# NethermindEth/zinc

Hardware: AMD Instinct MI355X
Metric: Zip commit+open MCoeffs/s at 2^24 witness (higher is better)
Workload: dtype i64

## Files before the change

zinc_amd/csrc/kernels_commit.cuh:

```cuda
#pragma once
#include <hip/hip_runtime.h>
#include <stdint.h>

#include "blake3.cuh"

namespace zipk {

typedef __int128 i128;
typedef unsigned __int128 u128;

#ifdef ZIPK_DEBUG_STAMPS
constexpr uint32_t kStampRec = 64;
__device__ __forceinline__ unsigned long long stamp_hw_id() {
    const uint32_t xcc = __builtin_amdgcn_s_getreg((3 << 11) | 20), hw = __builtin_amdgcn_s_getreg((31 << 11) | 4);
    return (unsigned long long)xcc | ((unsigned long long)hw << 8);
}
#endif

struct CommitArgs {
    const int64_t *evals;
    const uint32_t *perm1;
    const uint32_t *perm2;
    uint64_t *rows;
    uint32_t compact_rows;
    uint32_t *layers;
    uint32_t *roots;
    uint32_t row_len;
    uint32_t cw;
    uint32_t nact;
    uint32_t num_rows;
    uint32_t rounds_per_chunk;
    uint64_t chunk_ends;
    uint8_t *pk;
    uint32_t pk_stride, pk_off0, pk_off1, pk_off2;
    const uint32_t *pk_tab;
    uint32_t *chunk_done;
    uint32_t classes;
    const uint32_t *need;
    unsigned long long *clock;
    uint4 *slab;
#ifdef ZIPK_DEBUG_STAMPS
    unsigned long long *stamps;
#endif
};

__device__ __forceinline__ i128 shfl_up_i96(i128 x, int off) {
    uint32_t d0 = (uint32_t)x, d1 = (uint32_t)((u128)x >> 32), d2 = (uint32_t)((u128)x >> 64);
    d0 = __shfl_up(d0, off, 64);
    d1 = __shfl_up(d1, off, 64);
    d2 = __shfl_up(d2, off, 64);
    const int64_t hi = (int64_t)(int32_t)d2;
    return (i128)(((u128)(uint64_t)hi << 64) | ((u128)d1 << 32) | d0);
}

__device__ __forceinline__ void lds_barrier() {
    asm volatile("s_waitcnt lgkmcnt(0)\n\ts_barrier" ::: "memory");
}

template <int CTRL, int ROW_MASK>
__device__ __forceinline__ i128 dpp_i96(i128 x) {
    const int d0 = (int)(uint32_t)x, d1 = (int)(uint32_t)((u128)x >> 32), d2 = (int)(uint32_t)((u128)x >> 64);
    const uint32_t y0 = (uint32_t)__builtin_amdgcn_update_dpp(0, d0, CTRL, ROW_MASK, 0xF, false);
    const uint32_t y1 = (uint32_t)__builtin_amdgcn_update_dpp(0, d1, CTRL, ROW_MASK, 0xF, false);
    const uint32_t y2 = (uint32_t)__builtin_amdgcn_update_dpp(0, d2, CTRL, ROW_MASK, 0xF, false);
    const int64_t hi = (int64_t)(int32_t)y2;
    return (i128)(((u128)(uint64_t)hi << 64) | ((u128)y1 << 32) | y0);
}

__device__ __forceinline__ i128 block_exclusive_scan_i96(i128 total, i128 *wave_tot, int which) {
    const int lane = threadIdx.x & 63;
    const int wid = __builtin_amdgcn_readfirstlane((int)(threadIdx.x >> 6));
    i128 x = total;
    x += dpp_i96<0x111, 0xF>(x);
    x += dpp_i96<0x112, 0xF>(x);
    x += dpp_i96<0x114, 0xF>(x);
    x += dpp_i96<0x118, 0xF>(x);
    x += dpp_i96<0x142, 0xA>(x);
    x += dpp_i96<0x143, 0xC>(x);
    i128 *tot = wave_tot + 16 * which;
    if (lane == 63) tot[wid] = x;
    lds_barrier();
    i128 t = lane < 16 ? tot[lane] : (i128)0;
    t += dpp_i96<0x111, 0xF>(t);
    t += dpp_i96<0x112, 0xF>(t);
    t += dpp_i96<0x114, 0xF>(t);
    t += dpp_i96<0x118, 0xF>(t);
    i128 base = 0;
    if (wid > 0) {
        const uint32_t b0 = (uint32_t)__builtin_amdgcn_readlane((int)(uint32_t)t, wid - 1);
        const uint32_t b1 = (uint32_t)__builtin_amdgcn_readlane((int)(uint32_t)((u128)t >> 32), wid - 1);
        const uint32_t b2 = (uint32_t)__builtin_amdgcn_readlane((int)(uint32_t)((u128)t >> 64), wid - 1);
        base = (i128)(((u128)(uint64_t)(int64_t)(int32_t)b2 << 64) | ((u128)b1 << 32) | b0);
    }
    return base + (x - total);
}

__device__ __forceinline__ void store_hash(uint32_t *dst, const uint32_t (&h)[8]) {
    uint4 *d = reinterpret_cast<uint4 *>(dst);
    d[0] = make_uint4(h[0], h[1], h[2], h[3]);
    d[1] = make_uint4(h[4], h[5], h[6], h[7]);
}
__device__ __forceinline__ void load_hash(const uint32_t *src, uint32_t (&h)[8]) {
    const uint4 *s = reinterpret_cast<const uint4 *>(src);
    uint4 a = s[0], b = s[1];
    h[0] = a.x; h[1] = a.y; h[2] = a.z; h[3] = a.w;
    h[4] = b.x; h[5] = b.y; h[6] = b.z; h[7] = b.w;
}

__device__ __forceinline__ uint32_t level_off(uint32_t cw, uint32_t k) { return 2u * cw - ((2u * cw) >> k); }

template <bool ILV>
__device__ __forceinline__ uint32_t *tree_of(uint32_t *layers, uint32_t cw, uint32_t row) {
    return ILV ? layers + ((size_t)(row >> 2) * (2u * cw) * 4 + (row & 3u)) * 8 : layers + (size_t)row * (2u * cw) * 8;
}
template <bool ILV>
constexpr uint32_t kNodeWords = ILV ? 32u : 8u;

__device__ __forceinline__ uint32_t round_slot(uint32_t b, uint32_t G, uint32_t classes = 1) {
    if (G & 7u) return b;
    const uint32_t x = b & 7u, l = b >> 3;
    if (classes <= 1u) return x * (G >> 3) + l;
    const uint32_t per = (G >> 3) / classes, k = l / per;
    return k * (G / classes) + x * per + (l - k * per);
}
__device__ __forceinline__ uint32_t commit_class(uint32_t b, uint32_t G, uint32_t classes) {
    return classes <= 1u ? 0u : (b >> 3) / ((G >> 3) / classes);
}

template <int LVL, int E0, class Src>
__device__ __forceinline__ void subtree_hash(Src &src, uint32_t (&h)[8]) {
    if constexpr (LVL == 0) {
        src.template leaf<E0>(h);
    } else {
        uint32_t l[8], r[8];
        subtree_hash<LVL - 1, E0>(src, l);
        subtree_hash<LVL - 1, E0 + (1 << (LVL - 1))>(src, r);
        blake3_node(l, r, h);
        src.store(LVL, E0 >> LVL, h);
    }
}

constexpr int kStoreAll = 0, kStoreHinted = 1, kStorePacked = 3;

template <int E, int MODE = kStoreAll, bool LAZY = false>
struct StridedLeaves {
    static constexpr bool MASKED = MODE != kStoreAll;
    uint32_t w0[E], w1[E], w2[E];
    const uint64_t *lz_lo = nullptr;
    const uint32_t *lz_hi = nullptr;
    uint32_t lz_stride = 0;
    template <int E0>
    __device__ __forceinline__ void entry(uint32_t &a, uint32_t &b, uint32_t &c) const {
        if (LAZY) {
            const uint64_t lo = lz_lo[E0 * lz_stride];
            a = (uint32_t)lo;
            b = (uint32_t)(lo >> 32);
            c = lz_hi[E0 * lz_stride];
        } else {
            a = w0[E0];
            b = w1[E0];
            c = w2[E0];
        }
    }
    uint64_t *out_row;
    uint32_t *tree;
    uint32_t cw, T, tid;
    uint32_t base = 0;
    uint32_t compact = 0;
    uint32_t smask = 0xFFFFFFFFu;
    static constexpr uint32_t NW = MODE == kStorePacked ? 32u : 8u;
    uint8_t *pk_v = nullptr, *pk_n = nullptr;
    uint32_t pk_off0 = 0, pk_off1 = 0, pk_off2 = 0;
    __device__ __forceinline__ void set_packed(const CommitArgs &a, uint32_t row) {
        uint8_t *g = a.pk + (size_t)(row >> 2) * 4 * a.pk_stride;
        pk_v = g + (row & 3u) * 16u;
        pk_n = g + (row & 3u) * 32u;
        pk_off0 = 4u * a.pk_off0;
        pk_off1 = 4u * a.pk_off1;
        pk_off2 = 4u * a.pk_off2;
    }
    uint32_t ptab[16] = {};
    template <int K>
    __device__ __forceinline__ uint32_t pbase() const { return (ptab[K >> 1] >> ((K & 1) * 16)) & 0xFFFFu; }
    static __device__ __forceinline__ uint32_t lanes_below(uint64_t m) {
        return __builtin_amdgcn_mbcnt_hi((uint32_t)(m >> 32), __builtin_amdgcn_mbcnt_lo((uint32_t)m, 0u));
    }
    template <int E0>
    __device__ __forceinline__ void store_row_of(uint32_t d0, uint32_t d1, uint32_t d2) {
        if (MASKED && !(smask & (1u << E0))) return;
        const uint32_t j = base + E0 * T + tid;
        const uint32_t s = (uint32_t)((int32_t)d2 >> 31);
        if (MODE == kStorePacked) {
            const uint32_t pos = pbase<E0>() + lanes_below(__builtin_amdgcn_ballot_w64(true));
            *reinterpret_cast<uint4 *>(pk_v + (size_t)pos * 64) = make_uint4(d0, d1, d2, s);
        } else if (compact) {
            *reinterpret_cast<uint4 *>(out_row + (size_t)j * 2) = make_uint4(d0, d1, d2, s);
        } else {
            uint4 *o = reinterpret_cast<uint4 *>(out_row + (size_t)j * 4);
            o[0] = make_uint4(d0, d1, d2, s);
            o[1] = make_uint4(s, s, s, s);
        }
    }
    template <int E0>
    __device__ __forceinline__ void store_row() {
        uint32_t d0, d1, d2;
        entry<E0>(d0, d1, d2);
        store_row_of<E0>(d0, d1, d2);
    }
    template <int E0>
    __device__ __forceinline__ void leaf(uint32_t (&h)[8]) {
        uint32_t d0, d1, d2;
        entry<E0>(d0, d1, d2);
        store_row_of<E0>(d0, d1, d2);
        blake3_leaf_sext96(d0, d1, d2, h);
        if (!MASKED || (smask & (0x100u << E0))) {
            if (MODE == kStorePacked) {
                const uint32_t pos = pbase<8 + E0>() + lanes_below(__builtin_amdgcn_ballot_w64(true));
                store_hash(reinterpret_cast<uint32_t *>(pk_n + pk_off0) + (size_t)pos * 32, h);
            } else {
                store_hash(tree + (size_t)(base + E0 * T + tid) * 8, h);
            }
        }
    }
    template <int LVL, int E0>
    __device__ __forceinline__ void store(const uint32_t (&h)[8]) {
        if (MASKED && LVL <= 2 && !(smask & ((LVL == 1 ? 0x10000u : 0x1000000u) << (E0 >> LVL)))) return;
        const uint32_t e = E0 + (tid & ((1u << LVL) - 1u));
        const uint32_t n = (base + e * T + tid) >> LVL;
        if (MODE == kStorePacked && LVL == 1) {
            const uint64_t act = __builtin_amdgcn_ballot_w64(true);
            const bool odd = tid & 1u;
            const uint32_t pos = (odd ? pbase<16 + (E0 >> 1) * 2 + 1>() : pbase<16 + (E0 >> 1) * 2>()) +
                                 lanes_below(act & (odd ? 0xAAAAAAAAAAAAAAAAull : 0x5555555555555555ull));
            store_hash(reinterpret_cast<uint32_t *>(pk_n + pk_off1) + (size_t)pos * 32, h);
        } else if (MODE == kStorePacked && LVL == 2) {
            const uint64_t act = __builtin_amdgcn_ballot_w64(true);
            const uint32_t q = tid & 3u;
            constexpr int K0 = 24 + ((E0 >> 2) & 1) * 4;
            const uint32_t b01 = (q & 1u) ? pbase<K0 + 1>() : pbase<K0>(), b23 = (q & 1u) ? pbase<K0 + 3>() : pbase<K0 + 2>();
            const uint32_t pos = ((q & 2u) ? b23 : b01) + lanes_below(act & (0x1111111111111111ull << q));
            store_hash(reinterpret_cast<uint32_t *>(pk_n + pk_off2) + (size_t)pos * 32, h);
        } else {
            store_hash(tree + ((size_t)level_off(cw, LVL) + n) * NW, h);
        }
    }
};

template <int E>
__device__ __forceinline__ uint32_t store_mask(const uint32_t *need, uint32_t cw, uint32_t base, uint32_t T, uint32_t tid) {
    if (!need) return 0xFFFFFFFFu;
    const uint32_t *nv = need, *n0 = nv + (cw + 31) / 32, *n1 = n0 + (cw + 31) / 32, *n2 = n1 + (cw / 2 + 31) / 32;
    uint32_t m = 0;
#pragma unroll
    for (int e = 0; e < E; e++) {
        const uint32_t j = base + e * T + tid;
        m |= ((nv[j >> 5] >> (j & 31)) & 1u) << e;
        m |= ((n0[j >> 5] >> (j & 31)) & 1u) << (8 + e);
    }
#pragma unroll
    for (int g = 0; g < E / 2; g++) {
        const uint32_t i = (base + (2 * g + (tid & 1u)) * T + tid) >> 1;
        m |= ((n1[i >> 5] >> (i & 31)) & 1u) << (16 + g);
    }
#pragma unroll
    for (int g = 0; g < E / 4; g++) {
        const uint32_t i = (base + (4 * g + (tid & 3u)) * T + tid) >> 2;
        m |= ((n2[i >> 5] >> (i & 31)) & 1u) << (24 + g);
    }
    return m;
}

template <int E, int E0, class Src>
__device__ __forceinline__ void store_rows_only(Src &src) {
    if constexpr (E0 < E) {
        src.template store_row<E0>();
        store_rows_only<E, E0 + 1>(src);
    }
}

template <int LVL, int E0, class Src>
__device__ __forceinline__ void bfly_hash(Src &src, uint32_t (&h)[8]) {
    if constexpr (LVL == 0) {
        src.template leaf<E0>(h);
    } else {
        uint32_t A[8], B[8], m[16];
        bfly_hash<LVL - 1, E0>(src, A);
        bfly_hash<LVL - 1, E0 + (1 << (LVL - 1))>(src, B);
        const bool up = (src.tid >> (LVL - 1)) & 1;
#pragma unroll
        for (int i = 0; i < 8; i++) {
            const uint32_t snd = up ? A[i] : B[i];
            const uint32_t rcv = __shfl_xor(snd, 1 << (LVL - 1), 64);
            m[i] = up ? rcv : A[i];
            m[8 + i] = up ? B[i] : rcv;
        }
        blake3_block64(m, h);
        src.template store<LVL, E0>(h);
    }
}

template <bool ILV>
__device__ __forceinline__ void upper_stage(const CommitArgs &a, uint32_t first, uint32_t nrows_c, uint32_t lvl, uint32_t nl,
                                            uint32_t lane, uint32_t nlanes) {
    constexpr uint32_t NW = kNodeWords<ILV>;
    const uint32_t cw = a.cw, depth = 31u - __builtin_clz(cw);
    const uint32_t u_shift = depth - (lvl - 1u) - nl;
    const uint32_t total = nrows_c << u_shift;
    const uint32_t slot0 = round_slot(blockIdx.x, gridDim.x, a.classes);
    for (uint32_t idx = lane; idx < total; idx += nlanes) {
        const uint32_t ri = idx >> u_shift, i = idx & ((1u << u_shift) - 1u);
        const uint32_t r = slot0 + (first + ri) * gridDim.x;
        uint32_t *tree = tree_of<ILV>(a.layers, cw, r);
        const uint32_t *ch = tree + ((size_t)level_off(cw, lvl - 1u) + ((size_t)i << nl)) * NW;
        uint32_t c0[8], c1[8], h0[8];
        load_hash(ch, c0);
        load_hash(ch + NW, c1);
        if (nl == 1u) {
            blake3_node(c0, c1, h0);
            store_hash(tree + ((size_t)level_off(cw, lvl) + i) * NW, h0);
            if (lvl == depth) store_hash(a.roots + (size_t)r * 8, h0);
        } else {
            uint32_t c2[8], c3[8], h1[8], h2[8];
            blake3_node(c0, c1, h0);
            uint32_t *o = tree + ((size_t)level_off(cw, lvl) + 2u * i) * NW;
            store_hash(o, h0);
            asm volatile("" ::: "memory");
            load_hash(ch + 2 * NW, c2);
            load_hash(ch + 3 * NW, c3);
            blake3_node(c2, c3, h1);
            store_hash(o + NW, h1);
            blake3_node(h0, h1, h2);
            store_hash(tree + ((size_t)level_off(cw, lvl + 1u) + i) * NW, h2);
            if (lvl + 1u == depth) store_hash(a.roots + (size_t)r * 8, h2);
        }
    }
}

struct ChunkCursor {
    uint32_t first = 0, index = 0;
    __device__ __forceinline__ bool ends_with(const CommitArgs &a, uint32_t round, bool last) const {
        if (last) return true;
        if (a.chunk_ends) return (a.chunk_ends >> round) & 1u;
        return (round + 1) % a.rounds_per_chunk == 0;
    }
    __device__ __forceinline__ void advance(uint32_t round) {
        first = round + 1;
        index++;
    }
};

constexpr uint32_t kFinisherFlagWords = 16;

template <bool HASH, bool ILV = false>
struct ChunkFinisher {
    bool pending = false;
    uint32_t p_first = 0, p_nrows = 0, p_lvl = 0, p_index = 0;
    uint32_t p_base = 0;
    uint32_t n_deferred = 0;
    uint32_t *flags = nullptr;

    __device__ __forceinline__ void init(uint32_t *lds_flags, uint32_t tid) {
        flags = lds_flags;
        if (tid < kFinisherFlagWords) lds_flags[tid] = 0;
    }

    __device__ __forceinline__ void top_of_row() const {
        if (HASH && pending) asm volatile("s_waitcnt vmcnt(0)" ::: "memory");
    }

    static __device__ __forceinline__ void publish(const CommitArgs &a, uint32_t index, uint32_t lane) {
        if (!a.chunk_done) return;
        asm volatile("s_waitcnt vmcnt(0)" ::: "memory");
        if (lane == 0) {
            __builtin_amdgcn_fence(__ATOMIC_RELEASE, "agent");
            asm volatile("s_waitcnt vmcnt(0)" ::: "memory");
            __hip_atomic_fetch_add(&a.chunk_done[index], 1u, __ATOMIC_RELAXED, __HIP_MEMORY_SCOPE_AGENT);
        }
    }

    static __device__ __forceinline__ void signal(uint32_t *flag, uint32_t lane) {
        asm volatile("s_waitcnt vmcnt(0)" ::: "memory");
        if (lane == 0) __hip_atomic_fetch_add(flag, 1u, __ATOMIC_RELEASE, __HIP_MEMORY_SCOPE_WORKGROUP);
    }
    static __device__ __forceinline__ void wait_for(uint32_t *flag, uint32_t target) {
        uint32_t spins = 0;
        while (__hip_atomic_load(flag, __ATOMIC_ACQUIRE, __HIP_MEMORY_SCOPE_WORKGROUP) < target) {
            __builtin_amdgcn_s_sleep(2);
            if (++spins > (1u << 24)) __builtin_trap();
        }
    }

    static __device__ __forceinline__ bool stage_wide(uint32_t cw, uint32_t lvl, uint32_t nl, uint32_t j) {
        return j == 0u || (cw >> (lvl - 1u + nl)) >= 64u;
    }
    static __device__ __forceinline__ uint32_t stage_waves(uint32_t cw, uint32_t depth, uint32_t lvl0, uint32_t j, uint32_t W) {
        const uint32_t lvl = lvl0 + 2u * j;
        if (lvl > depth) return 0u;
        return stage_wide(cw, lvl, depth - lvl >= 1u ? 2u : 1u, j) ? W : 1u;
    }
    __device__ __forceinline__ uint32_t target(uint32_t cw, uint32_t depth, uint32_t j, uint32_t W) const {
        return (n_deferred - 1u) * stage_waves(cw, depth, p_base, j, W) + stage_waves(cw, depth, p_lvl, j, W);
    }
    __device__ __forceinline__ void after_hash(const CommitArgs &a, uint32_t wave, uint32_t lane, uint32_t T) {
        if (!(HASH && pending)) return;
        pending = false;
        n_deferred++;
        constexpr uint32_t kFinWaves = 8u;
        const uint32_t W = T >= 64u * kFinWaves ? kFinWaves : T >= 256u ? 4u : (T + 63u) / 64u;
        if (wave >= W) return;
        const uint32_t cw = a.cw, depth = 31u - __builtin_clz(cw);
        uint32_t lvl = p_lvl, j = 0, owner = 0;
        bool wide = true;
        while (lvl <= depth) {
            const uint32_t nl = depth - lvl >= 1u ? 2u : 1u;
            wide = stage_wide(cw, lvl, nl, j);
            if (wide) {
                if (j) wait_for(flags + (j - 1u), target(cw, depth, j - 1u, W));
                upper_stage<ILV>(a, p_first, p_nrows, lvl, nl, lane + 64u * wave, 64u * W);
                signal(flags + j, lane);
            } else {
                owner = j % W;
                if (wave == owner) {
                    wait_for(flags + (j - 1u), target(cw, depth, j - 1u, W));
                    upper_stage<ILV>(a, p_first, p_nrows, lvl, nl, lane, 64u);
                    signal(flags + j, lane);
                }
            }
            lvl += nl;
            j++;
        }
        if (j == 0u || wide) owner = 0u;
        if (wave == owner) {
            if (j && wide) wait_for(flags + (j - 1u), target(cw, depth, j - 1u, W));
            publish(a, p_index, lane);
        }
    }

    __device__ __forceinline__ void after_loop(const CommitArgs &a, uint32_t wave, uint32_t lane, uint32_t T, unsigned char *lds,
                                               uint32_t lds_bytes) {
        if (!(HASH && pending)) return;
        __syncthreads();
        const uint32_t cw = a.cw, depth = 31u - __builtin_clz(cw);
        const uint32_t tid = lane + 64u * wave;
        const uint32_t w_in0 = cw >> (p_lvl - 1u);
        const uint32_t n_in0 = p_nrows * w_in0;
        if (p_lvl <= depth && (n_in0 + n_in0 / 2u) * 32u <= lds_bytes && n_in0 >= 2u) {
            constexpr uint32_t NW = kNodeWords<ILV>;
            pending = false;
            uint4 *bufA = reinterpret_cast<uint4 *>(lds), *bufB = bufA + 2u * n_in0;
            const uint32_t slot0 = round_slot(blockIdx.x, gridDim.x, a.classes);
            const uint32_t sh0 = 31u - __builtin_clz(w_in0);
            for (uint32_t idx = tid; idx < n_in0; idx += T) {
                const uint32_t ri = idx >> sh0, i = idx & (w_in0 - 1u);
                const uint32_t r = slot0 + (p_first + ri) * gridDim.x;
                const uint4 *src = reinterpret_cast<const uint4 *>(tree_of<ILV>(a.layers, cw, r) + ((size_t)level_off(cw, p_lvl - 1u) + i) * NW);
                bufA[2u * idx] = src[0];
                bufA[2u * idx + 1u] = src[1];
            }
            __syncthreads();
            uint4 *in = bufA, *out = bufB;
            for (uint32_t lvl = p_lvl; lvl <= depth; lvl++) {
                const uint32_t w = cw >> lvl, sh = 31u - __builtin_clz(w), m = p_nrows * w;
                for (uint32_t idx = tid; idx < m; idx += T) {
                    const uint32_t ri = idx >> sh, i = idx & (w - 1u);
                    const uint32_t r = slot0 + (p_first + ri) * gridDim.x;
                    const uint4 a0 = in[4u * idx], a1 = in[4u * idx + 1u], b0 = in[4u * idx + 2u], b1 = in[4u * idx + 3u];
                    const uint32_t c0[8] = {a0.x, a0.y, a0.z, a0.w, a1.x, a1.y, a1.z, a1.w};
                    const uint32_t c1[8] = {b0.x, b0.y, b0.z, b0.w, b1.x, b1.y, b1.z, b1.w};
                    uint32_t h[8];
                    blake3_node(c0, c1, h);
                    store_hash(tree_of<ILV>(a.layers, cw, r) + ((size_t)level_off(cw, lvl) + i) * NW, h);
                    if (lvl == depth) store_hash(a.roots + (size_t)r * 8, h);
                    out[2u * idx] = make_uint4(h[0], h[1], h[2], h[3]);
                    out[2u * idx + 1u] = make_uint4(h[4], h[5], h[6], h[7]);
                }
                __syncthreads();
                uint4 *t = in;
                in = out;
                out = t;
            }
            if (wave == 0u) publish(a, p_index, lane);
            return;
        }
        after_hash(a, wave, lane, T);
    }

    __device__ __forceinline__ void chunk_end(const CommitArgs &a, uint32_t first_level, const ChunkCursor &cc, uint32_t round,
                                              bool last, uint32_t tid, uint32_t T) {
        const uint32_t wave = __builtin_amdgcn_readfirstlane(tid >> 6), lane = tid & 63u;
        if (!HASH) {
            if (a.chunk_done) {
                __syncthreads();
                if (wave == 0) publish(a, cc.index, lane);
            }
            return;
        }
        const uint32_t cw = a.cw, depth = 31u - __builtin_clz(cw);
        const uint32_t first = cc.first, nrows_c = round - first + 1;
        uint32_t lvl = first_level;
        const bool now = last || lvl > depth;
        if (now) {
            __syncthreads();
            if (lvl <= depth) {
                const uint32_t nl = depth - lvl >= 1u ? 2u : 1u;
                upper_stage<ILV>(a, first, nrows_c, lvl, nl, tid, T);
                lvl += nl;
            }
        }
        if (depth == 0 && tid == 0) {
            for (uint32_t ri = 0; ri < nrows_c; ri++) {
                const uint32_t r = round_slot(blockIdx.x, gridDim.x, a.classes) + (first + ri) * gridDim.x;
                uint32_t h[8];
                load_hash(a.layers + (size_t)r * (2u * cw) * 8, h);
                store_hash(a.roots + (size_t)r * 8, h);
            }
        }
        if (!last) p_base = lvl;
        pending = true;
        p_first = first;
        p_nrows = nrows_c;
        p_lvl = lvl;
        p_index = cc.index;
    }
};

__device__ __forceinline__ void stamp_clock(const CommitArgs &a, int slot) {
    if (a.clock && blockIdx.x == 0 && threadIdx.x == 0) {
        a.clock[2 * slot] = __builtin_amdgcn_s_memtime();
        a.clock[2 * slot + 1] = __builtin_amdgcn_s_memrealtime();
    }
}

__device__ __forceinline__ uint32_t opaque_zero(uint32_t dep) {
    uint32_t z;
    asm volatile("s_mov_b32 %0, 0" : "=s"(z) : "s"(dep));
    return z;
}

template <int E, bool HASH, int MODE = kStoreAll>
__global__ void __launch_bounds__(1024, 4) raa_commit_kernel(CommitArgs a) {
    constexpr bool MASKED = MODE != kStoreAll;
    extern __shared__ __align__(16) unsigned char smem[];
    constexpr int LOGE = (E == 1) ? 0 : (E == 2) ? 1 : (E == 4) ? 2 : 3;
    static_assert((1 << LOGE) == E && E <= 8, "E must be 1, 2, 4 or 8");

    const uint32_t tid0 = threadIdx.x, T = blockDim.x;
    constexpr uint32_t PAD = 32 / E;
    const uint32_t PS = T + PAD;
    const uint32_t cw = a.cw, row_len = a.row_len;
    const bool active = tid0 < a.nact;
    stamp_clock(a, 0);

    i128 *wave_tot = reinterpret_cast<i128 *>(smem);
    uint64_t *t2lo = reinterpret_cast<uint64_t *>(smem + 512);
    uint32_t *t2hi = reinterpret_cast<uint32_t *>(t2lo + E * PS);
    int64_t *rowbuf = reinterpret_cast<int64_t *>(t2hi + E * PS);
    uint32_t pidx[E];
    auto load_pidx = [&](uint32_t t) {
#pragma unroll
        for (int e = 0; e < E; e++) {
            uint32_t v1 = 0, v2 = 0;
            if (active) {
                v1 = a.perm1[t * E + e] & (row_len - 1);
                const uint32_t p2 = a.perm2[t * E + e];
                v2 = (p2 & (E - 1)) * PS + (p2 >> LOGE);
            }
            pidx[e] = v1 | (v2 << 16);
        }
    };
    load_pidx(tid0);
    const uint32_t smask = (MASKED && active) ? store_mask<E>(a.need, cw, 0u, a.nact, tid0) : 0xFFFFFFFFu;
    uint32_t ptab[16] = {};
    if (MODE == kStorePacked) {
        const uint32_t *wt = a.pk_tab + (size_t)__builtin_amdgcn_readfirstlane(tid0 >> 6) * 16;
#pragma unroll
        for (int k = 0; k < 16; k++) ptab[k] = __builtin_amdgcn_readfirstlane(wt[k]);
    }
    constexpr int NPF = (E >= 2) ? E / 2 : 1;
    const bool prefetch = row_len == NPF * T;
    int64_t nxt[NPF];

#ifdef ZIPK_DEBUG_STAMPS
    unsigned long long ph_a = 0, ph_b = 0, ph_c = 0, ph_t;
    if (tid0 == 0 && a.stamps) {
        a.stamps[(size_t)kStampRec * blockIdx.x] = wall_clock64();
        a.stamps[(size_t)kStampRec * blockIdx.x + 2] = stamp_hw_id();
    }
#define ZIPK_PH(acc) do { const unsigned long long now_ = wall_clock64(); acc += now_ - ph_t; ph_t = now_; } while (0)
#else
#define ZIPK_PH(acc) do { } while (0)
#endif
    uint32_t round = 0;
    ChunkCursor cc;
    if (a.classes > 1u) {
        const uint32_t c = commit_class(blockIdx.x, gridDim.x, a.classes);
        cc.index = c;
        const uint32_t prio = (a.classes - 1u - c) * 3u / (a.classes - 1u);
        if (prio == 3u) __builtin_amdgcn_s_setprio(3);
        else if (prio == 2u) __builtin_amdgcn_s_setprio(2);
        else if (prio == 1u) __builtin_amdgcn_s_setprio(1);
    }
    ChunkFinisher<HASH, MODE == kStorePacked> fin;
    fin.init(reinterpret_cast<uint32_t *>(rowbuf + row_len), tid0);
    const uint32_t wave0 = __builtin_amdgcn_readfirstlane(tid0 >> 6);
    for (uint32_t row = round_slot(blockIdx.x, gridDim.x, a.classes); row < a.num_rows; row += gridDim.x, round++) {
#ifdef ZIPK_DEBUG_STAMPS
        ph_t = wall_clock64();
#endif
        const uint32_t z = opaque_zero(row);
        const uint32_t tid = tid0 + z;
        const int64_t *in = a.evals + (size_t)row * row_len;
        uint64_t *out_row = a.rows + (size_t)row * cw * (a.compact_rows ? 2 : 4);

        const bool has_next = row + gridDim.x < a.num_rows;
        if (!(prefetch && round)) {
            if (round) lds_barrier();
            for (uint32_t i = tid; i < row_len; i += T) rowbuf[i] = in[i];
            lds_barrier();
        }
        if (prefetch && has_next) {
            const int64_t *nin = a.evals + (size_t)(row + gridDim.x) * row_len;
#pragma unroll
            for (int k = 0; k < NPF; k++) nxt[k] = nin[k * T + tid];
        }

        i128 v[E];
        if (active) {
#pragma unroll
            for (int e = 0; e < E; e++) v[e] = (i128)rowbuf[(pidx[e] ^ z) & 0xFFFFu];
#pragma unroll
            for (int e = 1; e < E; e++) v[e] += v[e - 1];
        } else {
#pragma unroll
            for (int e = 0; e < E; e++) v[e] = 0;
        }
        {
            const i128 pre = block_exclusive_scan_i96(v[E - 1], wave_tot, 0);
            if (active) {
#pragma unroll
                for (int e = 0; e < E; e++) {
                    v[e] += pre;
                    const uint32_t slot = e * PS + tid;
                    t2lo[slot] = (uint64_t)v[e];
                    t2hi[slot] = (uint32_t)((u128)v[e] >> 64);
                }
            }
        }
        lds_barrier();
        if (active) {
#pragma unroll
            for (int e = 0; e < E; e++) {
                const uint32_t slot = (pidx[e] ^ z) >> 16;
                const uint64_t lo = t2lo[slot];
                const int64_t hi = (int64_t)(int32_t)t2hi[slot];
                v[e] = (i128)(((u128)(uint64_t)hi << 64) | lo);
            }
#pragma unroll
            for (int e = 1; e < E; e++) v[e] += v[e - 1];
        }
        {
            const i128 pre = block_exclusive_scan_i96(v[E - 1], wave_tot, 1);
#pragma unroll
            for (int e = 0; e < E; e++) v[e] += pre;
        }

        if (active) {
#pragma unroll
            for (int e = 0; e < E; e++) {
                const uint32_t slot = e * PS + tid;
                t2lo[slot] = (uint64_t)v[e];
                t2hi[slot] = (uint32_t)((u128)v[e] >> 64);
            }
        }
        if (prefetch && has_next) {
#pragma unroll
            for (int k = 0; k < NPF; k++) rowbuf[k * T + tid] = nxt[k];
        }
        fin.top_of_row();
        lds_barrier();
        ZIPK_PH(ph_a);
        if (active) {
            StridedLeaves<E, MODE, true> src;
            src.out_row = out_row;
            src.compact = a.compact_rows;
            src.tree = HASH ? tree_of<MODE == kStorePacked>(a.layers, cw, row) : nullptr;
            src.cw = cw;
            src.T = a.nact;
            src.tid = tid;
            src.smask = smask;
            if (MODE == kStorePacked) {
                src.set_packed(a, row);
#pragma unroll
                for (int k = 0; k < 16; k++) src.ptab[k] = ptab[k];
            }
            {
                const uint32_t slot0 = (tid & (E - 1)) * PS + (tid >> LOGE);
                src.lz_lo = t2lo + slot0;
                src.lz_hi = t2hi + slot0;
                src.lz_stride = a.nact >> LOGE;
            }
            if (HASH) {
                uint32_t top[8];
                bfly_hash<LOGE, 0>(src, top);
            } else {
                store_rows_only<E, 0>(src);
            }
        }
        ZIPK_PH(ph_b);
        fin.after_hash(a, wave0, tid0 & 63u, T);
        const bool last = row + gridDim.x >= a.num_rows;
        if (cc.ends_with(a, round, last)) {
            fin.chunk_end(a, LOGE + 1, cc, round, last, tid, T);
            cc.advance(round);
        }
        ZIPK_PH(ph_c);
#ifdef ZIPK_DEBUG_STAMPS
        if (tid0 == 0 && a.stamps && round < kStampRec - 8) a.stamps[(size_t)kStampRec * blockIdx.x + 8 + round] = ph_t;
#endif
    }
    fin.after_loop(a, wave0, tid0 & 63u, T, smem + 512, (uint32_t)(E * PS * 12u));
    stamp_clock(a, 1);
#ifdef ZIPK_DEBUG_STAMPS
    if (tid0 == 0 && a.stamps) {
        unsigned long long *o = a.stamps + (size_t)kStampRec * blockIdx.x;
        o[1] = wall_clock64();
        o[3] = ph_a; o[4] = ph_b; o[5] = ph_c; o[6] = round;
    }
#endif
}

constexpr size_t c16_lds_bytes(uint32_t T) {
    return 512 + (size_t)16 * (T + 2) * 8 + (size_t)16 * (T + 2) + (size_t)T * 4 + 64;
}

template <int B, int P = 0>
__device__ __forceinline__ void transpose8_stage(uint32_t (&x)[8], bool up) {
    if constexpr (P < 4) {
        constexpr int r = ((P >> B) << (B + 1)) | (P & ((1 << B) - 1)), r2 = r | (1 << B);
        const uint32_t lo = x[r], hi = x[r2];
        const uint32_t rcv = __shfl_xor(up ? lo : hi, 1 << B, 64);
        x[r] = up ? rcv : lo;
        x[r2] = up ? hi : rcv;
        transpose8_stage<B, P + 1>(x, up);
    }
}
__device__ __forceinline__ void transpose8(uint32_t (&x)[8], uint32_t lane) {
    transpose8_stage<0>(x, lane & 1u);
    transpose8_stage<1>(x, (lane >> 1) & 1u);
    transpose8_stage<2>(x, (lane >> 2) & 1u);
}

template <uint32_t T, bool HASH, int MODE = kStoreAll>
__global__ void __launch_bounds__(T, 4) raa_commit16_kernel(CommitArgs a) {
    constexpr bool MASKED = MODE != kStoreAll;
    static_assert(MODE == kStoreAll || MODE == kStoreHinted || MODE == kStorePacked, "store mode");
    extern __shared__ __align__(16) unsigned char smem[];
    constexpr int E = 16;
    constexpr uint32_t PS = T + 2;
    const uint32_t tid0 = threadIdx.x;
    const uint32_t cw = a.cw, row_len = a.row_len;
    stamp_clock(a, 0);

    i128 *wave_tot = reinterpret_cast<i128 *>(smem);
    uint64_t *t2lo = reinterpret_cast<uint64_t *>(smem + 512);
    int8_t *t2dh = reinterpret_cast<int8_t *>(t2lo + (size_t)E * PS);
    int32_t *ghi = reinterpret_cast<int32_t *>(t2dh + (size_t)E * PS);
    uint64_t *park_lo = reinterpret_cast<uint64_t *>(smem + 512);
    uint32_t *park_hi = reinterpret_cast<uint32_t *>(park_lo + (size_t)8 * PS);

    const uint32_t smask0 = MASKED ? store_mask<8>(a.need, cw, 0u, 16u, (tid0 & ~7u) * 16u + (tid0 & 7u)) : 0xFFFFFFFFu;
    const uint32_t smask1 = MASKED ? store_mask<8>(a.need, cw, 0u, 16u, (tid0 & ~7u) * 16u + 8u + (tid0 & 7u)) : 0xFFFFFFFFu;
    uint32_t ptab0[16] = {}, ptab1[16] = {};
    if (MODE == kStorePacked) {
        const uint32_t *wt = a.pk_tab + (size_t)__builtin_amdgcn_readfirstlane(tid0 >> 6) * 32;
#pragma unroll
        for (int k = 0; k < 16; k++) {
            ptab0[k] = __builtin_amdgcn_readfirstlane(wt[k]);
            ptab1[k] = __builtin_amdgcn_readfirstlane(wt[16 + k]);
        }
    }

    uint32_t round = 0;
    ChunkCursor cc;
    ChunkFinisher<HASH, MODE == kStorePacked> fin;
    fin.init(reinterpret_cast<uint32_t *>(ghi + T), tid0);
    const uint32_t wave0 = __builtin_amdgcn_readfirstlane(tid0 >> 6);
    for (uint32_t row = round_slot(blockIdx.x, gridDim.x, a.classes); row < a.num_rows; row += gridDim.x, round++) {
        fin.top_of_row();
        const uint32_t z = opaque_zero(row);
        const uint32_t tid = tid0 + z;
        const int64_t *in = a.evals + (size_t)row * row_len;
        uint64_t *out_row = a.rows + (size_t)row * cw * (a.compact_rows ? 2 : 4);

        uint32_t p2[E];
        i128 v[E];
        {
            const uint4 *q1 = reinterpret_cast<const uint4 *>(a.perm1 + (size_t)tid * E);
            const uint4 *q2 = reinterpret_cast<const uint4 *>(a.perm2 + (size_t)tid * E);
#pragma unroll
            for (int k = 0; k < E / 4; k++) {
                const uint4 s1 = q1[k], s2 = q2[k];
                v[4 * k + 0] = (i128)in[s1.x & (row_len - 1)];
                v[4 * k + 1] = (i128)in[s1.y & (row_len - 1)];
                v[4 * k + 2] = (i128)in[s1.z & (row_len - 1)];
                v[4 * k + 3] = (i128)in[s1.w & (row_len - 1)];
                p2[4 * k + 0] = s2.x;
                p2[4 * k + 1] = s2.y;
                p2[4 * k + 2] = s2.z;
                p2[4 * k + 3] = s2.w;
            }
        }
#pragma unroll
        for (int e = 1; e < E; e++) v[e] += v[e - 1];
        {
            const i128 pre = block_exclusive_scan_i96(v[E - 1], wave_tot, 0);
            const int32_t phi = (int32_t)(uint32_t)((u128)pre >> 64);
            ghi[tid] = phi;
#pragma unroll
            for (int e = 0; e < E; e++) {
                const i128 t = v[e] + pre;
                t2lo[e * PS + tid] = (uint64_t)t;
                t2dh[e * PS + tid] = (int8_t)((int32_t)(uint32_t)((u128)t >> 64) - phi);
            }
        }
        lds_barrier();
#pragma unroll
        for (int e = 0; e < E; e++) {
            const uint32_t j = p2[e];
            const uint32_t slot = (j & 15u) * PS + (j >> 4);
            const uint64_t lo = t2lo[slot];
            const int64_t hi = (int64_t)(ghi[j >> 4] + (int32_t)t2dh[slot]);
            v[e] = (i128)(((u128)(uint64_t)hi << 64) | lo);
        }
#pragma unroll
        for (int e = 1; e < E; e++) v[e] += v[e - 1];
        {
            const i128 pre = block_exclusive_scan_i96(v[E - 1], wave_tot, 1);
#pragma unroll
            for (int e = 0; e < E; e++) v[e] += pre;
        }
#pragma unroll
        for (int e = 8; e < E; e++) {
            park_lo[(e - 8) * PS + tid] = (uint64_t)v[e];
            park_hi[(e - 8) * PS + tid] = (uint32_t)((u128)v[e] >> 64);
        }
        uint32_t x0[8], x1[8], x2[8];
#pragma unroll
        for (int e = 0; e < 8; e++) {
            x0[e] = (uint32_t)(uint64_t)v[e];
            x1[e] = (uint32_t)((uint64_t)v[e] >> 32);
            x2[e] = (uint32_t)((u128)v[e] >> 64);
        }
#pragma unroll
        for (uint32_t q = 0; q < 2; q++) {
            if (q) {
#pragma unroll
                for (int e = 0; e < 8; e++) {
                    const uint64_t lo = park_lo[e * PS + tid];
                    x0[e] = (uint32_t)lo;
                    x1[e] = (uint32_t)(lo >> 32);
                    x2[e] = park_hi[e * PS + tid];
                }
            }
            transpose8(x0, tid);
            transpose8(x1, tid);
            transpose8(x2, tid);
            StridedLeaves<8, MODE> src;
            if (MODE == kStorePacked) {
                src.set_packed(a, row);
#pragma unroll
                for (int k = 0; k < 16; k++) src.ptab[k] = q ? ptab1[k] : ptab0[k];
            }
            src.out_row = out_row;
            src.compact = a.compact_rows;
            src.tree = HASH ? tree_of<MODE == kStorePacked>(a.layers, cw, row) : nullptr;
            src.cw = cw;
            src.T = 16;
            src.tid = (tid & ~7u) * 16u + q * 8u + (tid & 7u);
            src.smask = q ? smask1 : smask0;
#pragma unroll
            for (int e = 0; e < 8; e++) {
                src.w0[e] = x0[e];
                src.w1[e] = x1[e];
                src.w2[e] = x2[e];
            }
            if (HASH) {
                uint32_t top[8];
                bfly_hash<3, 0>(src, top);
            } else {
                store_rows_only<8, 0>(src);
            }
        }
        fin.after_hash(a, wave0, tid0 & 63u, T);
        const bool last = row + gridDim.x >= a.num_rows;
        if (cc.ends_with(a, round, last)) {
            fin.chunk_end(a, 4u, cc, round, last, tid, T);
            cc.advance(round);
        }
    }
    fin.after_loop(a, wave0, tid0 & 63u, T, smem + 512, (uint32_t)(E * PS * 9u));
    stamp_clock(a, 1);
}

constexpr uint32_t kSlabThreads = 1024;
constexpr size_t cslab_lds_bytes() {
    return 512 + (size_t)kSlabThreads * 32 + 4 * kFinisherFlagWords;
}

__device__ __forceinline__ void vmem_barrier() {
    asm volatile("s_waitcnt vmcnt(0)" ::: "memory");
    __syncthreads();
}

__device__ __forceinline__ i128 slab_get(const uint4 &u) {
    const int64_t hi = (int64_t)(int32_t)u.z;
    return (i128)(((u128)(uint64_t)hi << 64) | ((u128)u.y << 32) | u.x);
}

template <int E, bool HASH>
__global__ void __launch_bounds__(kSlabThreads, 4) raa_commit_slab_kernel(CommitArgs a) {
    constexpr uint32_t T = kSlabThreads;
    constexpr int LOGE = (E == 32) ? 5 : 6;
    static_assert((1 << LOGE) == E, "E must be 32 or 64");
    extern __shared__ __align__(16) unsigned char smem[];
    const uint32_t tid0 = threadIdx.x;
    const uint32_t cw = a.cw, row_len = a.row_len;
    stamp_clock(a, 0);

    i128 *wave_tot = reinterpret_cast<i128 *>(smem);
    i128 *pre1 = reinterpret_cast<i128 *>(smem + 512);
    i128 *runp = pre1 + T;
    uint4 *slab = a.slab + (size_t)blockIdx.x * cw;

    uint32_t round = 0;
    ChunkCursor cc;
    ChunkFinisher<HASH> fin;
    fin.init(reinterpret_cast<uint32_t *>(runp + T), tid0);
    const uint32_t wave0 = __builtin_amdgcn_readfirstlane(tid0 >> 6);
    for (uint32_t row = round_slot(blockIdx.x, gridDim.x, a.classes); row < a.num_rows; row += gridDim.x, round++) {
        const uint32_t z = opaque_zero(row);
        const uint32_t tid = tid0 + z;
        const int64_t *in = a.evals + (size_t)row * row_len;
        if (round) __syncthreads();

        i128 s = 0;
        {
            const uint4 *q1 = reinterpret_cast<const uint4 *>(a.perm1 + (size_t)tid * E);
#pragma unroll 2
            for (int k = 0; k < E / 4; k++) {
                const uint4 p = q1[k];
                const uint32_t idx[4] = {p.x, p.y, p.z, p.w};
#pragma unroll
                for (int i = 0; i < 4; i++) {
                    s += (i128)in[idx[i] & (row_len - 1)];
                    const u128 u = (u128)s;
                    slab[(size_t)(4 * k + i) * T + tid] = make_uint4((uint32_t)u, (uint32_t)(u >> 32), (uint32_t)(u >> 64), 0u);
                }
            }
        }
        pre1[tid] = block_exclusive_scan_i96(s, wave_tot, 0);
        vmem_barrier();

        const uint4 *q2 = reinterpret_cast<const uint4 *>(a.perm2 + (size_t)tid * E);
        s = 0;
#pragma unroll 2
        for (int k = 0; k < E / 4; k++) {
            const uint4 p = q2[k];
            const uint32_t idx[4] = {p.x, p.y, p.z, p.w};
#pragma unroll
            for (int i = 0; i < 4; i++) {
                const uint32_t j = idx[i];
                s += slab_get(slab[(size_t)(j & (E - 1)) * T + (j >> LOGE)]) + pre1[j >> LOGE];
            }
        }
        runp[tid] = block_exclusive_scan_i96(s, wave_tot, 1);

#pragma unroll 1
        for (uint32_t q = 0; q < (uint32_t)E / 8u; q++) {
            const uint32_t tq = tid + opaque_zero(q);
            uint32_t x0[8], x1[8], x2[8];
            {
                i128 run = runp[tq];
                const uint4 *q2q = reinterpret_cast<const uint4 *>(a.perm2 + (size_t)tq * E) + 2 * q;
                const uint4 pa = q2q[0], pb = q2q[1];
                const uint32_t idx[8] = {pa.x, pa.y, pa.z, pa.w, pb.x, pb.y, pb.z, pb.w};
#pragma unroll
                for (int e = 0; e < 8; e++) {
                    const uint32_t j = idx[e];
                    run += slab_get(slab[(size_t)(j & (E - 1)) * T + (j >> LOGE)]) + pre1[j >> LOGE];
                    const u128 u = (u128)run;
                    x0[e] = (uint32_t)u;
                    x1[e] = (uint32_t)(u >> 32);
                    x2[e] = (uint32_t)(u >> 64);
                }
                runp[tq] = run;
            }
            transpose8(x0, tq);
            transpose8(x1, tq);
            transpose8(x2, tq);
            StridedLeaves<8> src;
            src.out_row = a.rows + (size_t)row * cw * (a.compact_rows ? 2 : 4);
            src.compact = a.compact_rows;
            src.tree = HASH ? tree_of<false>(a.layers, cw, row) : nullptr;
            src.cw = cw;
            src.T = E;
            src.tid = (tq & ~7u) * (uint32_t)E + q * 8u + (tq & 7u);
#pragma unroll
            for (int e = 0; e < 8; e++) {
                src.w0[e] = x0[e];
                src.w1[e] = x1[e];
                src.w2[e] = x2[e];
            }
            if (HASH) {
                uint32_t top[8];
                bfly_hash<3, 0>(src, top);
            } else {
                store_rows_only<8, 0>(src);
            }
        }
        fin.after_hash(a, wave0, tid0 & 63u, T);
        const bool last = row + gridDim.x >= a.num_rows;
        if (cc.ends_with(a, round, last)) {
            fin.chunk_end(a, 4u, cc, round, last, tid, T);
            cc.advance(round);
        }
    }
    fin.after_loop(a, wave0, tid0 & 63u, T, smem + 512, (uint32_t)(T * 32u));
    stamp_clock(a, 1);
}

__global__ void __launch_bounds__(256) witness_digest_kernel(const uint64_t *w, uint64_t n, unsigned long long *out) {
    unsigned long long a = 0, b = 0;
    const uint64_t n2 = n / 2, stride = (uint64_t)gridDim.x * blockDim.x;
    const ulonglong2 *w2 = reinterpret_cast<const ulonglong2 *>(w);
    uint64_t i = (uint64_t)blockIdx.x * blockDim.x + threadIdx.x;
    for (; i + 3 * stride < n2; i += 4 * stride) {
        ulonglong2 v[4];
#pragma unroll
        for (int k = 0; k < 4; k++) v[k] = w2[i + k * stride];
#pragma unroll
        for (int k = 0; k < 4; k++) {
            const uint64_t j = 2 * (i + k * stride);
            a += v[k].x + v[k].y;
            b += v[k].x * (2ull * j + 1ull) + v[k].y * (2ull * j + 3ull);
        }
    }
    for (; i < n2; i += stride) {
        const ulonglong2 v = w2[i];
        a += v.x + v.y;
        b += v.x * (4ull * i + 1ull) + v.y * (4ull * i + 3ull);
    }
    if ((n & 1) && blockIdx.x == 0 && threadIdx.x == 0) {
        a += w[n - 1];
        b += w[n - 1] * (2ull * (n - 1) + 1ull);
    }
    for (int off = 32; off > 0; off >>= 1) {
        a += __shfl_down(a, off, 64);
        b += __shfl_down(b, off, 64);
    }
    if ((threadIdx.x & 63) == 0) {
        atomicAdd(out, a);
        atomicAdd(out + 1, b);
    }
}

__global__ void __launch_bounds__(256) expand_rows_kernel(const uint4 *in, uint4 *out, uint64_t n) {
    for (uint64_t i = (uint64_t)blockIdx.x * blockDim.x + threadIdx.x; i < n; i += (uint64_t)gridDim.x * blockDim.x) {
        const uint4 v = in[i];
        out[2 * i] = v;
        out[2 * i + 1] = make_uint4(v.w, v.w, v.w, v.w);
    }
}

__global__ void __launch_bounds__(64) wait_counter_kernel(uint32_t *counter, uint32_t target, uint32_t zero,
                                                          uint32_t *timeout_flag, unsigned long long timeout_ticks) {
    __builtin_amdgcn_s_setprio(3);
    if (threadIdx.x == 0) {
        const unsigned long long t0 = wall_clock64();
        while (__hip_atomic_fetch_add(counter, zero, __ATOMIC_RELAXED, __HIP_MEMORY_SCOPE_AGENT) < target) {
            __builtin_amdgcn_s_sleep(64);
            if (wall_clock64() - t0 > timeout_ticks) {
                __hip_atomic_store(timeout_flag, 1u, __ATOMIC_RELAXED, __HIP_MEMORY_SCOPE_SYSTEM);
                break;
            }
        }
        __builtin_amdgcn_fence(__ATOMIC_ACQUIRE, "agent");
    }
}

struct UpperNodes {
    const uint32_t *in;
    uint32_t *tree, *root;
    uint32_t cw, level_in, depth, n0;
    template <int E0>
    __device__ __forceinline__ void leaf(uint32_t (&h)[8]) {
        load_hash(in + (size_t)E0 * 8, h);
    }
    __device__ __forceinline__ void store(int lvl, uint32_t idx, const uint32_t (&h)[8]) {
        const uint32_t lv = level_in + lvl;
        store_hash(tree + ((size_t)level_off(cw, lv) + (n0 >> lvl) + idx) * 8, h);
        if (lv == depth) store_hash(root, h);
    }
};

template <int NL>
__global__ void __launch_bounds__(256) merkle_upper_kernel(uint32_t *layers, uint32_t *roots,
                                                           uint32_t num_rows, uint32_t cw,
                                                           uint32_t level_in, uint32_t depth) {
    const uint32_t width_in = cw >> level_in;
    const uint32_t groups = width_in >> NL;
    const uint32_t log_groups = 31u - __builtin_clz(groups);
    const uint32_t gid = blockIdx.x * blockDim.x + threadIdx.x;
    if (gid >= num_rows * groups) return;
    const uint32_t r = gid >> log_groups, g = gid & (groups - 1);
    uint32_t *tree = layers + (size_t)r * (2u * cw) * 8;
    const uint32_t *src_nodes = tree + ((size_t)level_off(cw, level_in) + ((size_t)g << NL)) * 8;
    UpperNodes src{src_nodes, tree, roots + (size_t)r * 8, cw, level_in, depth, g << NL};
    uint32_t top[8];
    subtree_hash<NL, 0>(src, top);
}

__global__ void copy_roots_depth0_kernel(const uint32_t *layers, uint32_t *roots, uint32_t num_rows,
                                         uint32_t cw) {
    const uint32_t r = blockIdx.x * blockDim.x + threadIdx.x;
    if (r >= num_rows) return;
    const uint32_t *tree = layers + (size_t)r * (2u * cw) * 8;
#pragma unroll
    for (int i = 0; i < 8; i++) roots[(size_t)r * 8 + i] = tree[i];
}

template <int LIMBS>
__global__ void __launch_bounds__(256) merkle_leaves_kernel(const uint64_t *leaves, uint32_t *layers,
                                                            uint32_t num_trees, uint32_t nleaves) {
    const size_t gid = (size_t)blockIdx.x * blockDim.x + threadIdx.x;
    if (gid >= (size_t)num_trees * nleaves) return;
    const uint32_t t = (uint32_t)(gid / nleaves), i = (uint32_t)(gid % nleaves);
    uint64_t limb[LIMBS];
#pragma unroll
    for (int k = 0; k < LIMBS; k++) limb[k] = leaves[gid * LIMBS + k];
    uint32_t h[8];
    blake3_leaf_limbs<LIMBS>(limb, h);
    store_hash(layers + ((size_t)t * (2u * nleaves) + i) * 8, h);
}

}
```

Baseline: 11340.

## Collapse narrow Merkle top levels into one wave-level shuffle reduction

When the upper Merkle stages become too narrow for all finisher waves, the finisher now processes the remaining top levels in a single pass per 64-lane group. It hashes a 4-leaf subtree per lane, then climbs the rest of the tree with ds_bpermute shuffles in registers instead of running a separate stage, with its own flag wait, for each level. Groups are spread over the finisher waves, and completion is counted on a dedicated top flag before publish. This cuts per-level synchronisation and global round-trips in the serial tail. The cost is extra shuffle traffic and some idle lanes, plus more complex flag accounting.

```diff
diff --git a/zinc_amd/csrc/kernels_commit.cuh b/zinc_amd/csrc/kernels_commit.cuh
--- a/zinc_amd/csrc/kernels_commit.cuh
+++ b/zinc_amd/csrc/kernels_commit.cuh
@@ -299,6 +299,34 @@
     }
 }
 
+__device__ __forceinline__ uint32_t opaque_zero(uint32_t dep) {
+    uint32_t z;
+    asm volatile("s_mov_b32 %0, 0" : "=s"(z) : "s"(dep));
+    return z;
+}
+
+template <bool ILV>
+__device__ __forceinline__ void subtree4(const CommitArgs &a, uint32_t *tree, uint32_t r, uint32_t lvl, uint32_t i,
+                                         uint32_t (&h2)[8]) {
+    constexpr uint32_t NW = kNodeWords<ILV>;
+    const uint32_t cw = a.cw, depth = 31u - __builtin_clz(cw);
+    const uint32_t *ch = tree + ((size_t)level_off(cw, lvl - 1u) + ((size_t)i << 2)) * NW;
+    uint32_t c0[8], c1[8], c2[8], c3[8], h0[8], h1[8];
+    load_hash(ch, c0);
+    load_hash(ch + NW, c1);
+    blake3_node(c0, c1, h0);
+    uint32_t *o = tree + ((size_t)level_off(cw, lvl) + 2u * i) * NW;
+    store_hash(o, h0);
+    asm volatile("" ::: "memory");
+    load_hash(ch + 2 * NW, c2);
+    load_hash(ch + 3 * NW, c3);
+    blake3_node(c2, c3, h1);
+    store_hash(o + NW, h1);
+    blake3_node(h0, h1, h2);
+    store_hash(tree + ((size_t)level_off(cw, lvl + 1u) + i) * NW, h2);
+    if (lvl + 1u == depth) store_hash(a.roots + (size_t)r * 8, h2);
+}
+
 template <bool ILV>
 __device__ __forceinline__ void upper_stage(const CommitArgs &a, uint32_t first, uint32_t nrows_c, uint32_t lvl, uint32_t nl,
                                             uint32_t lane, uint32_t nlanes) {
@@ -311,27 +339,52 @@
         const uint32_t ri = idx >> u_shift, i = idx & ((1u << u_shift) - 1u);
         const uint32_t r = slot0 + (first + ri) * gridDim.x;
         uint32_t *tree = tree_of<ILV>(a.layers, cw, r);
-        const uint32_t *ch = tree + ((size_t)level_off(cw, lvl - 1u) + ((size_t)i << nl)) * NW;
-        uint32_t c0[8], c1[8], h0[8];
-        load_hash(ch, c0);
-        load_hash(ch + NW, c1);
+        uint32_t h[8];
         if (nl == 1u) {
-            blake3_node(c0, c1, h0);
-            store_hash(tree + ((size_t)level_off(cw, lvl) + i) * NW, h0);
-            if (lvl == depth) store_hash(a.roots + (size_t)r * 8, h0);
+            const uint32_t *ch = tree + ((size_t)level_off(cw, lvl - 1u) + ((size_t)i << 1)) * NW;
+            uint32_t c0[8], c1[8];
+            load_hash(ch, c0);
+            load_hash(ch + NW, c1);
+            blake3_node(c0, c1, h);
+            store_hash(tree + ((size_t)level_off(cw, lvl) + i) * NW, h);
+            if (lvl == depth) store_hash(a.roots + (size_t)r * 8, h);
         } else {
-            uint32_t c2[8], c3[8], h1[8], h2[8];
-            blake3_node(c0, c1, h0);
-            uint32_t *o = tree + ((size_t)level_off(cw, lvl) + 2u * i) * NW;
-            store_hash(o, h0);
-            asm volatile("" ::: "memory");
-            load_hash(ch + 2 * NW, c2);
-            load_hash(ch + 3 * NW, c3);
-            blake3_node(c2, c3, h1);
-            store_hash(o + NW, h1);
-            blake3_node(h0, h1, h2);
-            store_hash(tree + ((size_t)level_off(cw, lvl + 1u) + i) * NW, h2);
-            if (lvl + 1u == depth) store_hash(a.roots + (size_t)r * 8, h2);
+            subtree4<ILV>(a, tree, r, lvl, i, h);
+        }
+    }
+}
+
+template <bool ILV>
+__device__ __forceinline__ void narrow_top(const CommitArgs &a, uint32_t first, uint32_t units, uint32_t lvl, uint32_t g,
+                                           uint32_t lane0) {
+    constexpr uint32_t NW = kNodeWords<ILV>;
+    const uint32_t cw = a.cw, depth = 31u - __builtin_clz(cw);
+    const uint32_t slot0 = round_slot(blockIdx.x, gridDim.x, a.classes);
+    const uint32_t lane = lane0 + opaque_zero(g);
+    const uint32_t l1 = lvl + 1u;
+    const uint32_t k0 = 64u * g;
+    uint32_t n = units - k0 < 64u ? units - k0 : 64u;
+    uint32_t x[8] = {};
+    if (lane < n) {
+        const uint32_t sh = depth - l1, k = k0 + lane;
+        const uint32_t r = slot0 + (first + (k >> sh)) * gridDim.x;
+        subtree4<ILV>(a, tree_of<ILV>(a.layers, cw, r), r, lvl, k & ((1u << sh) - 1u), x);
+    }
+    for (uint32_t l = l1 + 1u; l <= depth; l++) {
+        n >>= 1;
+        uint32_t c0[8], c1[8];
+        const int s0 = (int)((8u * lane) & 252u);
+#pragma unroll
+        for (int i = 0; i < 8; i++) {
+            c0[i] = (uint32_t)__builtin_amdgcn_ds_bpermute(s0, (int)x[i]);
+            c1[i] = (uint32_t)__builtin_amdgcn_ds_bpermute(s0 + 4, (int)x[i]);
+        }
+        blake3_node(c0, c1, x);
+        if (lane < n) {
+            const uint32_t sh = depth - l, k = (k0 >> (l - l1)) + lane;
+            const uint32_t r = slot0 + (first + (k >> sh)) * gridDim.x;
+            store_hash(tree_of<ILV>(a.layers, cw, r) + ((size_t)level_off(cw, l) + (k & ((1u << sh) - 1u))) * NW, x);
+            if (l == depth) store_hash(a.roots + (size_t)r * 8, x);
         }
     }
 }
@@ -357,6 +410,7 @@
     uint32_t p_first = 0, p_nrows = 0, p_lvl = 0, p_index = 0;
     uint32_t p_base = 0;
     uint32_t n_deferred = 0;
+    uint32_t top_waves = 0;
     uint32_t *flags = nullptr;
 
     __device__ __forceinline__ void init(uint32_t *lds_flags, uint32_t tid) {
@@ -390,6 +444,7 @@
         }
     }
 
+    static constexpr uint32_t kTopFlag = kFinisherFlagWords - 1u;
     static __device__ __forceinline__ bool stage_wide(uint32_t cw, uint32_t lvl, uint32_t nl, uint32_t j) {
         return j == 0u || (cw >> (lvl - 1u + nl)) >= 64u;
     }
@@ -420,18 +475,28 @@
                 signal(flags + j, lane);
             } else {
                 owner = j % W;
-                if (wave == owner) {
+                const uint32_t units = nl == 2u ? p_nrows << (depth - lvl - 1u) : 0u;
+                const uint32_t ngroups = nl == 2u ? (units + 63u) / 64u : 1u;
+                top_waves += ngroups < W ? ngroups : W;
+                const uint32_t g0 = (wave + W - owner) % W;
+                if (g0 < ngroups) {
                     wait_for(flags + (j - 1u), target(cw, depth, j - 1u, W));
-                    upper_stage<ILV>(a, p_first, p_nrows, lvl, nl, lane, 64u);
-                    signal(flags + j, lane);
+                    if (nl == 2u) {
+                        for (uint32_t g = g0; g < ngroups; g += W) narrow_top<ILV>(a, p_first, units, lvl, g, lane);
+                    } else {
+                        upper_stage<ILV>(a, p_first, p_nrows, lvl, nl, lane, 64u);
+                    }
+                    signal(flags + kTopFlag, lane);
                 }
+                break;
             }
             lvl += nl;
             j++;
         }
         if (j == 0u || wide) owner = 0u;
         if (wave == owner) {
-            if (j && wide) wait_for(flags + (j - 1u), target(cw, depth, j - 1u, W));
+            if (!wide) wait_for(flags + kTopFlag, top_waves);
+            else if (j) wait_for(flags + (j - 1u), target(cw, depth, j - 1u, W));
             publish(a, p_index, lane);
         }
     }
@@ -531,12 +596,6 @@
     }
 }
 
-__device__ __forceinline__ uint32_t opaque_zero(uint32_t dep) {
-    uint32_t z;
-    asm volatile("s_mov_b32 %0, 0" : "=s"(z) : "s"(dep));
-    return z;
-}
-
 template <int E, bool HASH, int MODE = kStoreAll>
 __global__ void __launch_bounds__(1024, 4) raa_commit_kernel(CommitArgs a) {
     constexpr bool MASKED = MODE != kStoreAll;
```

Result: no change. 11290 (-0.4%).
